# chanchanchan97/ICAFusion

Measured on NVIDIA H100. Metric: 640x512 RGB+IR pairs/sec end-to-end, higher is better.
Workload: dtype f16

## Files before the change

icafusion_b200/_lib.py:

```python
from __future__ import annotations

import ctypes as C
import os

_HERE = os.path.dirname(os.path.abspath(__file__))
LIB_PATH = os.path.join(_HERE, "libicaf_b200.so")

ACT_NONE, ACT_SILU, ACT_GELU = 0, 1, 2
EPI_BIAS_ROW, EPI_ADD_RES, EPI_SCALED_RES, EPI_LN_FOLD, EPI_EMIT_STATS = 1, 2, 4, 8, 16


class ConvGeom(C.Structure):
    _fields_ = [(n, C.c_int) for n in ("B", "Hi", "Wi", "Cin", "Ho", "Wo", "Cout", "kh", "kw", "stride", "pad",
                                       "k_pad", "w_rows", "act", "epi")]


class ConvIO(C.Structure):
    _fields_ = [("x", C.c_void_p), ("x_ld", C.c_int64), ("w", C.c_void_p), ("bias", C.c_void_p),
                ("res", C.c_void_p), ("res_ld", C.c_int64), ("y", C.c_void_p), ("y_ld", C.c_int64),
                ("alpha", C.c_void_p), ("beta", C.c_void_p),
                ("ln_stats", C.c_void_p), ("ln_colsum", C.c_void_p), ("ln_parts", C.c_int), ("ln_eps", C.c_float),
                ("stats_out", C.c_void_p)]


class ConvPlan(C.Structure):
    _fields_ = [(n, C.c_int) for n in ("kernel", "bn", "a_mode", "tile_w", "tile_h", "tiles_x", "tiles_y", "cblk", "halo",
                                       "stages", "splits", "grid_x", "grid_y", "grid_z", "cluster", "smem_bytes",
                                       "work_items", "ctas")]


class LossHyp(C.Structure):
    _fields_ = [(n, C.c_float) for n in ("box", "obj", "cls", "cls_pw", "obj_pw", "anchor_t", "fl_gamma", "gr", "cp", "cn")] + \
               [("balance", C.c_float * 5)]


class AugTile(C.Structure):
    _fields_ = [("rgb", C.c_void_p), ("ir", C.c_void_p)] + \
               [(n, C.c_int) for n in ("H0", "W0", "h", "w", "x1a", "y1a", "x2a", "y2a", "x1b", "y1b", "xtab", "ytab")]


class AugSample(C.Structure):
    _fields_ = [("tile", AugTile * 4)] + [(n, C.c_int) for n in ("ntiles", "canvas", "warp", "flipud", "fliplr", "reserved")] + \
               [("lut", C.c_uint8 * (2 * 3 * 256))]


KERNEL_TC = 0

_vp, _i, _i64, _f = C.c_void_p, C.c_int, C.c_int64, C.c_float
SIGNATURES = {
    "icaf_version": [],
    "icaf_last_error": [],
    "icaf_sm_count": [],
    "icaf_kernel_launches": [],
    "icaf_conv2d_fwd": [C.POINTER(ConvGeom), C.POINTER(ConvIO), _i, _vp],
    "icaf_conv2d_plan": [C.POINTER(ConvGeom), _i, _i, _i, C.POINTER(ConvPlan)],
    "icaf_conv2d_fwd_simt": [C.POINTER(ConvGeom), C.POINTER(ConvIO), _i, _vp],
    "icaf_pack_image": [_vp, _i, _f, _i, _i, _i, _vp, _vp],
    "icaf_pack_image_s2d": [_vp, _i, _f, _i, _i, _i, _vp, _vp],
    "icaf_letterbox": [_vp, _i, _i, _i, _vp, _i, _i, _i, _i, _i, _i, _vp, _vp, _i, _vp],
    "icaf_sppf_pool": [_vp, _i64, _vp, _vp, _vp, _i64, _i, _i, _i, _i, _vp],
    "icaf_upsample2x": [_vp, _i64, _vp, _i64, _i, _i, _i, _i, _vp],
    "icaf_copy_channels": [_vp, _i64, _vp, _i64, _i64, _i, _vp],
    "icaf_prefetch_l2": [_vp, C.c_size_t, _vp],
    "icaf_dmff_pool_tokens": [_vp, _vp, _i64, _vp, _vp, _vp, _vp, _vp, _vp, _vp, _i, _i, _i, _i, _i, _i, _i, _vp],
    "icaf_row_stats": [_vp, _vp, _vp, _vp, _i64, _i, _vp],
    "icaf_layernorm": [_vp, _vp, _vp, _vp, _vp, _vp, _vp, _vp, _i64, _i, _f, _vp],
    "icaf_cross_attention": [_vp, _vp, _vp, _vp, _vp, _vp, _i, _i, _i, _i, _i, _vp],
    "icaf_cross_attention_simt": [_vp, _vp, _vp, _vp, _vp, _vp, _i, _i, _i, _i, _i, _vp],
    "icaf_dmff_upsample_cat": [_vp, _vp, _i, _vp, _vp, _i64, _vp, _i64, _i, _i, _i, _i, _i, _i, _i, _vp],
    "icaf_nms_workspace_bytes": [_i, _i],
    "icaf_nms": [_vp, _i, _i, _i, _f, _f, _i, C.c_uint64, _i, _vp, _vp, _vp, C.c_size_t, _vp],
    "icaf_loss_workspace_bytes": [_i, _i, _i, C.POINTER(C.c_int), C.POINTER(C.c_int), _i, _i],
    "icaf_compute_loss_fwd": [C.POINTER(C.c_void_p), _i, _i, C.POINTER(C.c_int), C.POINTER(C.c_int), _i, _i, _i, _i, _vp, _i,
                              C.POINTER(C.c_float), C.POINTER(LossHyp), _vp, _vp, C.c_size_t, _vp],
    "icaf_compute_loss_bwd": [C.POINTER(C.c_void_p), _i, _i, C.POINTER(C.c_int), C.POINTER(C.c_int), _i, _i, _i, _i, _vp, _i,
                              C.POINTER(C.c_float), C.POINTER(LossHyp), _vp, C.POINTER(C.c_void_p), _vp, C.c_size_t, _vp],
    "icaf_conv2d_wgrad_workspace_bytes": [C.POINTER(ConvGeom)],
    "icaf_conv2d_wgrad": [C.POINTER(ConvGeom), _vp, _i64, _vp, _i64, _vp, _f, _i, _vp, C.c_size_t, _vp],
# ... 21 lines not shown
    "icaf_augment": [_vp, C.c_size_t, _i, _i, _i, _vp, _vp, _vp],
}

_lib = None


class IcafError(RuntimeError):
    pass


def lib() -> C.CDLL:
    global _lib
    if _lib is None:
        if not os.path.exists(LIB_PATH):
            raise IcafError(f"{LIB_PATH} not found -- build it with `python -m icafusion_b200.build`; "
                            "icafusion_b200 has no non-CUDA fallback")
        L = C.CDLL(LIB_PATH)
        for name, argtypes in SIGNATURES.items():
            fn = getattr(L, name)
            fn.argtypes = argtypes
            fn.restype = {"icaf_last_error": C.c_char_p, "icaf_kernel_launches": C.c_longlong,
                          "icaf_nms_workspace_bytes": C.c_size_t, "icaf_loss_workspace_bytes": C.c_size_t,
                          "icaf_conv2d_wgrad_workspace_bytes": C.c_size_t, "icaf_train_workspace_bytes": C.c_size_t,
                          "icaf_cross_attention_bwd_workspace_bytes": C.c_size_t,
                          "icaf_augment_params_bytes": C.c_size_t}.get(name, C.c_int)
        _lib = L
    return _lib


def check(rc: int, what: str = "") -> None:
    if rc != 0:
        msg = lib().icaf_last_error()
        raise IcafError(f"{what or 'icaf call'} failed (code {rc}): {msg.decode() if msg else '?'}")
```

icafusion_b200/csrc/conv_common.cuh:

```cuda
#pragma once
#include "icaf_internal.cuh"

namespace icaf {

constexpr int BM = 128;
constexpr int BK = 64;
constexpr int kLag = 2;
constexpr int kThreads = 288;

enum AMode { A_GATHER = 0, A_TMA2D = 1, A_TMA4D = 2 };

struct ConvProblem {
  const __half* x; const float* bias; const __half* res; __half* y;
  const float* alpha; const float* beta;
  long long x_ld, res_ld, y_ld;
  const float2* ln_stats;
  const float* ln_s;
  float2* stats_out;
};
struct ConvParams {
  ConvProblem p[2];
  int M, N, K, k_pad;
  int B, Hi, Wi, Cin, Ho, Wo, kh, kw, stride, pad;
  int act, epi;
  int a_mode, tw, th, tiles_x, tiles_y;
  int stages;
  int splits;
  int cblk;
  int ln_parts;
  float ln_eps, ln_inv_k;
  int m_tiles, n_tiles, tiles;
  int tma_epi;
};
struct ConvMaps {
  CUtensorMap w[2];
  CUtensorMap a[2];
  CUtensorMap y[2];
  CUtensorMap res[2];
};

__device__ __forceinline__ ConvProblem pick_problem(const ConvParams& P, unsigned z) {
  ConvProblem r;
  r.x = z ? P.p[1].x : P.p[0].x;          r.bias = z ? P.p[1].bias : P.p[0].bias;
  r.res = z ? P.p[1].res : P.p[0].res;    r.y = z ? P.p[1].y : P.p[0].y;
  r.alpha = z ? P.p[1].alpha : P.p[0].alpha; r.beta = z ? P.p[1].beta : P.p[0].beta;
  r.x_ld = z ? P.p[1].x_ld : P.p[0].x_ld; r.res_ld = z ? P.p[1].res_ld : P.p[0].res_ld;
  r.y_ld = z ? P.p[1].y_ld : P.p[0].y_ld;
  r.ln_stats = z ? P.p[1].ln_stats : P.p[0].ln_stats; r.ln_s = z ? P.p[1].ln_s : P.p[0].ln_s;
  r.stats_out = z ? P.p[1].stats_out : P.p[0].stats_out;
  return r;
}

struct TileOrigin { int m0, tb, oy0, ox0; };
__device__ __forceinline__ void tile_origin(const ConvParams& P, int mtile, int& m0, int& tb, int& oy0, int& ox0) {
  m0 = mtile * BM; tb = 0; oy0 = 0; ox0 = 0;
// ... 273 lines not shown
template <int BN>
__device__ __forceinline__ void tma_load_tile(const ConvParams& P, const CUtensorMap* map, uint32_t s, uint32_t bar, int n0,
                                              const TileOrigin& o) {
  const int halves = (BN == 128 && n0 + 64 < P.N) ? 2 : 1;
  const uint32_t half_bytes = P.a_mode == A_TMA4D ? uint32_t(P.tw * P.th) * 128u : uint32_t(kOutHalfBytes);
  mbar_arrive_expect_tx(bar, uint32_t(halves) * half_bytes);
  for (int hh = 0; hh < halves; ++hh) {
    const uint32_t dst = s + uint32_t(hh * kOutHalfBytes);
    if (P.a_mode == A_TMA4D) tma_load_4d(dst, map, bar, n0 + 64 * hh, o.ox0, o.oy0, o.tb);
    else tma_load_2d(dst, map, bar, n0 + 64 * hh, o.m0);
  }
}

struct ConvPlan {
  int kernel;
  int bn;
  unsigned grid_x, grid_y, grid_z, cluster;
  int smem;
  int tiles, m_tiles, n_tiles;
  int sms;
  bool persist;
  bool xm;
  int ctas;
};

}
```

icafusion_b200/csrc/conv_gemm.cu:

```cuda
#include <cstdlib>
#include <cstring>

#include "conv_common.cuh"

namespace icaf {

constexpr int kMaxStages = 10;
template <int BN>
struct SmemLayout {
  static constexpr int kABytes = BM * BK * 2;
  static constexpr int kBBytes = BN * BK * 2;
  static constexpr int kStageBytes = kABytes + kBBytes;
  static constexpr int kPitch = BN + 4;
  static constexpr int kAccBytes = BM * kPitch * 4;
  static constexpr int kTailBytes = 256 + BN * 4 + 1024;
  __host__ __device__ static int region(int stages) { return stages * kStageBytes > kAccBytes ? stages * kStageBytes : kAccBytes; }
  static int total(int stages) { return region(stages) + kTailBytes; }
};


template <int BN, bool kTmaA>
__device__ __forceinline__ void load_stage(const ConvParams& P, int a_mode, uint32_t sa, uint32_t bar, uint32_t bytes,
                                           const CUtensorMap* mw, const CUtensorMap* ma, int kb, int n0, const TileOrigin& o) {
  mbar_arrive_expect_tx(bar, bytes);
// ... 234 lines not shown
    if (elect_one()) {
      const CUtensorMap* mw = bz ? &maps.w[1] : &maps.w[0];
      const CUtensorMap* ma = bz ? &maps.a[1] : &maps.a[0];
      const uint32_t a_bytes = a_mode == A_TMA2D ? L::kABytes : (a_mode == A_TMA4D ? uint32_t(P.tw * P.th) * 128u : 0u);
      const uint32_t bytes = L::kBBytes + a_bytes;
      int s = 0;
      uint32_t ph = 0;
      for (int kb = 0; kb < nkb; ++kb) {
        mbar_wait_quiet(empty_bar(s), ph ^ 1);
        load_stage<BN, false>(P, a_mode, smem_base + s * L::kStageBytes, full_bar(s), bytes, mw, ma, kb_begin + kb, n0, o);
        if (++s == kStages) { s = 0; ph ^= 1; }
      }
      if (tma_epi && has_res) {
        mbar_wait_quiet(empty_bar(s), ph ^ 1);
        tma_load_tile<BN>(P, bz ? &maps.res[1] : &maps.res[0], smem_base + uint32_t(s) * L::kStageBytes, res_bar, n0, o);
      }
    }
    __syncwarp();
    if (splits > 1) { cluster_arrive(); cluster_wait(); cluster_arrive(); cluster_wait(); }
  }
}

constexpr int kPersistThreads = 384;
struct PersistLayout {
  static constexpr int kStageBytes = SmemLayout<128>::kStageBytes;
  static constexpr int kOutBytes = 2 * kOutHalfBytes;
  static constexpr int kPitch = 32 + 4;
  static constexpr int kChunkBytes = BM * kPitch * 4;
  static_assert(kChunkBytes <= kOutBytes, "the XM staged chunk lives in the output tile");
  __host__ __device__ static int bar_off(int stages) { return stages * kStageBytes + 2 * kOutBytes; }
  static int total(int stages) { return bar_off(stages) + 256 + 2 * 128 * 4 + 1024; }
};

struct PersistTile { int z, n0; TileOrigin o; };
__device__ __forceinline__ PersistTile persist_tile(const ConvParams& P, int t) {
  PersistTile pt;
  const int r = t / P.n_tiles;
  const int mtile = r % P.m_tiles;
  pt.n0 = (t - r * P.n_tiles) * 128;
  pt.z = r / P.m_tiles;
  tile_origin(P, mtile, pt.o.m0, pt.o.tb, pt.o.oy0, pt.o.ox0);
  return pt;
}

template <int CC>
__device__ __forceinline__ void stage_chunk(const float (&acc0)[64], const float (&acc1)[64], float* sacc, int w, int l) {
#pragma unroll
  for (int i = 16 * CC; i < 16 * CC + 16; i += 2) {
    const int r = 16 * w + (l >> 2) + 8 * ((i >> 1) & 1), col = 8 * (i >> 2) - 32 * CC + 2 * (l & 3);
    *reinterpret_cast<float2*>(sacc + r * PersistLayout::kPitch + col) = make_float2(acc0[i], acc0[i + 1]);
    *reinterpret_cast<float2*>(sacc + (r + 64) * PersistLayout::kPitch + col) = make_float2(acc1[i], acc1[i + 1]);
  }
}

template <bool XM>
__global__ void __launch_bounds__(kPersistThreads, 1)
conv_gemm_persist_kernel(const ConvParams P, const __grid_constant__ ConvMaps maps) {
  extern __shared__ uint8_t smem_raw[];
  const uint32_t smem_base = (smem_u32(smem_raw) + 1023u) & ~1023u;
  using L = SmemLayout<128>;
  using PL = PersistLayout;
  const int kStages = P.stages;
  const uint32_t bar_off = uint32_t(PL::bar_off(kStages));
  const uint32_t bar_base = smem_base + bar_off;
  auto full_bar = [&](int s) { return bar_base + 8u * s; };
// ... 18 lines not shown
    mbar_init(res_bar(0), 1);
    mbar_init(res_bar(1), 1);
    fence_mbar_init();
  }
  if (tid == 32) {
    tma_prefetch_desc(&maps.w[0]);
    tma_prefetch_desc(&maps.a[0]);
    if (P.tiles > P.m_tiles * P.n_tiles) { tma_prefetch_desc(&maps.w[1]); tma_prefetch_desc(&maps.a[1]); }
    if (!XM) {
      tma_prefetch_desc(&maps.y[0]);
      if (has_res) tma_prefetch_desc(&maps.res[0]);
    }
  }
  __syncthreads();
  pdl_wait();

  if (wg == 0) {
    setmaxnreg_dec<40>();
    if (tid < 32 && elect_one()) {
      const uint32_t a_bytes = a_mode == A_TMA2D ? L::kABytes : uint32_t(P.tw * P.th) * 128u;
      const uint32_t bytes = L::kBBytes + a_bytes;
      int s = 0;
      uint32_t ph = 0;
      for (int tile = blockIdx.x; tile < P.tiles; tile += gridDim.x) {
        const PersistTile pt = persist_tile(P, tile);
        const CUtensorMap* mw = pt.z ? &maps.w[1] : &maps.w[0];
        const CUtensorMap* ma = pt.z ? &maps.a[1] : &maps.a[0];
        for (int kb = 0; kb < nkb; ++kb) {
          mbar_wait_quiet(empty_bar(s), ph ^ 1);
          load_stage<128, true>(P, a_mode, smem_base + s * L::kStageBytes, full_bar(s), bytes, mw, ma, kb, pt.n0, pt.o);
          if (++s == kStages) { s = 0; ph ^= 1; }
        }
      }
    }
    return;
  }

  setmaxnreg_inc<232>();
  const int c = wg - 1;
  const int t = tid & 127, w = t >> 5, l = t & 31;
  const int bar_id = 2 + c;
  const uint32_t sout = smem_base + uint32_t(kStages * L::kStageBytes + c * PL::kOutBytes);
  float* sacc = reinterpret_cast<float*>(smem_gen + kStages * L::kStageBytes + c * PL::kOutBytes);
  float* sbias = reinterpret_cast<float*>(smem_gen + bar_off + 256 + c * 128 * 4);
  for (int tile = blockIdx.x + c * gridDim.x; tile < P.tiles; tile += 2 * gridDim.x) {
    const int j = (tile - int(blockIdx.x)) / int(gridDim.x);
    const PersistTile pt = persist_tile(P, tile);
    const ConvProblem pr = pick_problem(P, pt.z);
    const int n0 = pt.n0;
    const TileOrigin& o = pt.o;
    const float bias_r = (pr.bias && !(P.epi & ICAF_EPI_BIAS_ROW) && n0 + t < P.N) ? __ldg(pr.bias + n0 + t) : 0.f;
    float alpha = 0.f, beta = 1.f;
    if (P.epi & ICAF_EPI_SCALED_RES) { alpha = __ldg(pr.alpha); beta = __ldg(pr.beta); }
    StagedRow sr;
    float rb[4] = {0.f, 0.f, 0.f, 0.f};
    if (XM) {
      staged_row<128, XM>(sr, P, pr, o, t, n0);
    } else {
      fragment_row_bias(rb, P, pr, o, w, l);
      if (t == 0) {
        bulk_wait_group_read<0>();
        if (has_res) tma_load_tile<128>(P, pt.z ? &maps.res[1] : &maps.res[0], sout, res_bar(c), n0, o);
      }
      sbias[t] = bias_r;
      named_bar_sync(bar_id, 128);
    }

    float acc0[64], acc1[64];
#pragma unroll
    for (int i = 0; i < 64; ++i) { acc0[i] = 0.f; acc1[i] = 0.f; }
    auto hand_back = [&](int s) { if (l == 0) mbar_arrive(empty_bar(s)); };
    const int g0 = j * nkb;
    const int s0 = g0 % kStages;
    const uint32_t ph0 = uint32_t(g0 / kStages) & 1u;
    if (j > 0) mbar_wait_quiet(order_bar(c), uint32_t((j >> 1) - (1 - c)) & 1u);
    const int s_last = mma_loop<128>(acc0, acc1, smem_base, kStages, nkb, s0, ph0, full_bar, hand_back);
    if (l == 0) mbar_arrive(order_bar(c ^ 1));
    wgmma_wait<0>();
    hand_back(s_last);

    if constexpr (!XM) {
      if (has_res) mbar_wait_quiet(res_bar(c), uint32_t(j >> 1) & 1u);
      epi_tile_fragments<64>(epi_mode_act<false>(P, has_res), acc0, acc1, sout, sbias, rb, alpha, beta, w, l);
      fence_proxy_async_smem();
      named_bar_sync(bar_id, 128);
      if (t == 0) {
        tma_store_tile<128>(P, pt.z ? &maps.y[1] : &maps.y[0], sout, n0, o);
        if (tile + 2 * int(gridDim.x) >= P.tiles) bulk_wait_group<0>();
      }
      continue;
    }

    const int mode_act = epi_mode_act<XM>(P, has_res);
    const float* arow = sacc + size_t(t) * PL::kPitch;
#pragma unroll 1
    for (int cc = 0; cc < 4; ++cc) {
      named_bar_sync(bar_id, 128);
      if (cc == 0) sbias[t] = bias_r;
      switch (cc) {
        case 0: stage_chunk<0>(acc0, acc1, sacc, w, l); break;
        case 1: stage_chunk<1>(acc0, acc1, sacc, w, l); break;
        case 2: stage_chunk<2>(acc0, acc1, sacc, w, l); break;
        default: stage_chunk<3>(acc0, acc1, sacc, w, l); break;
      }
      named_bar_sync(bar_id, 128);
      const int cb = 32 * cc;
      if (sr.mvalid && n0 + cb < P.N) {
        uint32_t acc[32];
        load_staged(acc, arow);
        epi_staged_chunk<XM>(mode_act, acc, sr, sbias, alpha, beta, cb, n0 + cb, P.N);
      }
// ... 37 lines not shown
  if (!g || n_io < 1 || n_io > 2) return set_error(ICAF_ERR_BAD_ARG, "conv2d: need 1 or 2 problems");
  if (!(g->Cin == 4 || g->Cin % 8 == 0)) return set_error(ICAF_ERR_UNSUPPORTED, "conv2d: Cin must be 4 or a multiple of 8");
  if (g->Cin == 4 && (g->Wi % 2 || g->stride % 2 || g->pad % 2 || g->kw % 2))
    return set_error(ICAF_ERR_UNSUPPORTED, "conv2d: packed-image (Cin=4) path needs even Wi, stride, pad, kw");
  if (g->k_pad % 64 || g->k_pad < g->kh * g->kw * g->Cin) return set_error(ICAF_ERR_BAD_ARG, "conv2d: bad k_pad");
  if (g->w_rows < g->Cout) return set_error(ICAF_ERR_BAD_ARG, "conv2d: w_rows < Cout");
  long long M = (long long)g->B * g->Ho * g->Wo;
  if (M <= 0 || M > 0x7fffffffLL || (long long)g->B * g->Hi * g->Wi > 0x7fffffffLL)
    return set_error(ICAF_ERR_BAD_ARG, "conv2d: size out of range");
  if ((g->epi & (ICAF_EPI_ADD_RES | ICAF_EPI_SCALED_RES)) == (ICAF_EPI_ADD_RES | ICAF_EPI_SCALED_RES))
    return set_error(ICAF_ERR_BAD_ARG, "conv2d: ADD_RES and SCALED_RES are exclusive");
  if ((g->epi & ICAF_EPI_LN_FOLD) && ((g->epi & ~ICAF_EPI_LN_FOLD) != 0 || !(g->act == ICAF_ACT_NONE || g->act == ICAF_ACT_GELU) ||
                                      g->kh != 1 || g->kw != 1 || g->stride != 1 || g->pad != 0))
    return set_error(ICAF_ERR_UNSUPPORTED, "conv2d: LN_FOLD is a linear-layer (1x1) epilogue without residual, activation none / GELU");
  if ((g->epi & ICAF_EPI_EMIT_STATS) && ((g->epi & ~ICAF_EPI_EMIT_STATS) != ICAF_EPI_SCALED_RES || g->act != ICAF_ACT_NONE))
    return set_error(ICAF_ERR_UNSUPPORTED, "conv2d: EMIT_STATS rides on the SCALED_RES epilogue without activation");
  P.M = int(M); P.N = g->Cout; P.K = g->kh * g->kw * g->Cin; P.k_pad = g->k_pad;
  P.B = g->B; P.Hi = g->Hi; P.Wi = g->Wi; P.Cin = g->Cin; P.Ho = g->Ho; P.Wo = g->Wo;
  P.kh = g->kh; P.kw = g->kw; P.stride = g->stride; P.pad = g->pad; P.act = g->act; P.epi = g->epi;
  P.a_mode = A_GATHER; P.tw = P.th = P.tiles_x = P.tiles_y = 0; P.stages = 2; P.splits = 1; P.cblk = 64;
  P.ln_parts = 0; P.ln_eps = 0.f; P.ln_inv_k = 0.f;
  P.m_tiles = P.n_tiles = P.tiles = 0;
  P.tma_epi = 0;
  memset(P.p, 0, sizeof(P.p));
  return ICAF_OK;
}

static int fill_params(const icaf_conv_geom* g, const icaf_conv_io* io, int n_io, ConvParams& P, const __half* (&w)[2]) {
  if (!io) return set_error(ICAF_ERR_BAD_ARG, "conv2d: null io");
  if (int rc = fill_geom(g, n_io, P)) return rc;
  for (int i = 0; i < 2; ++i) {
    const icaf_conv_io& s = io[i < n_io ? i : 0];
    bool need_res = g->epi & (ICAF_EPI_ADD_RES | ICAF_EPI_SCALED_RES);
    if (!s.x || !s.w || !s.y || (need_res && !s.res) || ((g->epi & ICAF_EPI_SCALED_RES) && (!s.alpha || !s.beta)))
      return set_error(ICAF_ERR_BAD_ARG, "conv2d: null pointer");
    if ((reinterpret_cast<uintptr_t>(s.x) & 15) || (reinterpret_cast<uintptr_t>(s.w) & 15) || (s.x_ld % 8 && g->Cin != 4) ||
        (g->Cin == 4 && s.x_ld != 4))
      return set_error(ICAF_ERR_BAD_ARG, "conv2d: x / w must be 16-byte aligned with x_ld a multiple of 8");
    if ((g->epi & ICAF_EPI_LN_FOLD) && (!s.ln_stats || !s.ln_colsum || s.ln_parts < 1 || s.ln_parts > 64))
      return set_error(ICAF_ERR_BAD_ARG, "conv2d: LN_FOLD needs ln_stats, ln_colsum and 1..64 partials per row");
    if ((g->epi & ICAF_EPI_EMIT_STATS) && !s.stats_out) return set_error(ICAF_ERR_BAD_ARG, "conv2d: EMIT_STATS needs stats_out");
    if (i > 0 && (g->epi & ICAF_EPI_LN_FOLD) && (s.ln_parts != io[0].ln_parts || s.ln_eps != io[0].ln_eps))
      return set_error(ICAF_ERR_BAD_ARG, "conv2d: grouped problems must share ln_parts / ln_eps");
    P.p[i] = ConvProblem{(const __half*)s.x, s.bias, need_res ? (const __half*)s.res : nullptr, (__half*)s.y, s.alpha, s.beta,
                         s.x_ld, s.res_ld, s.y_ld,
                         (g->epi & ICAF_EPI_LN_FOLD) ? (const float2*)s.ln_stats : nullptr,
// ... 48 lines not shown
  if (tiles * 2 <= pl.sms && nkb >= 8) {
    splits = int(pl.sms / tiles);
    if (splits > 8) splits = 8;
    if (splits > nkb / 4) splits = nkb / 4;
    if (splits < 1) splits = 1;
  }
  if (splits > 1) {
    const int per = (nkb + splits - 1) / splits;
    if (stages > per) stages = per < 2 ? 2 : per;
    gx *= splits;
  }
  if (stages > kMaxStages || L::total(stages) > kSmemCap)
    return set_error(ICAF_ERR_BAD_ARG, "conv2d(tc): shared-memory plan exceeds the ring / 227 KB");
  P.stages = stages;
  P.splits = splits;
  pl.kernel = ICAF_KERNEL_TC; pl.bn = BN;
  pl.grid_x = gx; pl.grid_y = gy; pl.grid_z = gz; pl.cluster = unsigned(splits);
  pl.smem = L::total(stages);
  pl.tiles = int(tiles); pl.m_tiles = mt; pl.n_tiles = int(gy);
  pl.persist = false; pl.ctas = int(gx * gy * gz);
  return ICAF_OK;
}

static int plan_persist(ConvParams& P, ConvPlan& pl) {
  constexpr int kSmemCap = 227 * 1024;
  int stages = kMaxStages;
  while (stages > 2 && PersistLayout::total(stages) > kSmemCap) --stages;
  if (PersistLayout::total(stages) > kSmemCap)
    return set_error(ICAF_ERR_BAD_ARG, "conv2d(persist): shared-memory plan exceeds 227 KB");
  P.stages = stages;
  P.m_tiles = pl.m_tiles; P.n_tiles = pl.n_tiles; P.tiles = pl.tiles;
  pl.persist = true;
  pl.ctas = pl.tiles < pl.sms ? pl.tiles : pl.sms;
  pl.smem = PersistLayout::total(stages);
  return ICAF_OK;
}

template <int BN>
static int encode_maps(const ConvParams& P, const __half* const (&w)[2], const icaf_conv_geom* g, int n_io, bool out_maps,
                       ConvMaps& maps) {
  memset(&maps, 0, sizeof(maps));
  for (int i = 0; i < n_io; ++i) {
    int rc = encode_tmap_2d(&maps.w[i], w[i], (uint64_t)P.k_pad, (uint64_t)g->w_rows, (uint64_t)P.k_pad * 2, BK, BN);
    if (rc) return rc;
    const ConvProblem& pr = P.p[i];
    if (P.a_mode == A_TMA2D)
      rc = encode_tmap_2d(&maps.a[i], pr.x, (uint64_t)P.Cin, (uint64_t)P.M, (uint64_t)pr.x_ld * 2, BK, BM);
    else if (P.a_mode == A_TMA4D)
      rc = encode_tmap_nhwc(&maps.a[i], pr.x, P.Cin, P.Wi, P.Hi, P.B, pr.x_ld, BK, P.tw * P.stride, P.th * P.stride, P.stride,
                            P.stride);
    if (rc) return rc;
    if (out_maps) {
      auto out_map = [&](CUtensorMap* m, const __half* base, long long ld) {
        return P.a_mode != A_TMA4D ? encode_tmap_2d(m, base, (uint64_t)P.N, (uint64_t)P.M, (uint64_t)ld * 2, 64, BM)
                                   : encode_tmap_nhwc(m, base, P.N, P.Wo, P.Ho, P.B, ld, 64, P.tw, P.th, 1, 1);
      };
      if ((rc = out_map(&maps.y[i], pr.y, pr.y_ld))) return rc;
      if (pr.res && (rc = out_map(&maps.res[i], pr.res, pr.res_ld))) return rc;
    }
  }
  if (n_io == 1) { maps.w[1] = maps.w[0]; maps.a[1] = maps.a[0]; maps.y[1] = maps.y[0]; maps.res[1] = maps.res[0]; }
  return ICAF_OK;
}

template <int BN>
static int launch_conv(const ConvParams& P, const ConvPlan& pl, const __half* const (&w)[2], const icaf_conv_geom* g, int n_io,
                       cudaStream_t st) {
  void (*kernel)(ConvParams, ConvMaps) = pl.xm ? conv_gemm_tc_kernel<BN, true> : conv_gemm_tc_kernel<BN, false>;
  if (pl.persist) kernel = pl.xm ? conv_gemm_persist_kernel<true> : conv_gemm_persist_kernel<false>;
  static bool configured[2][2][kMaxDevices] = {};
  if (int rc = configure_smem(kernel, 227 * 1024, configured[pl.persist][pl.xm], "conv2d: cudaFuncSetAttribute")) return rc;
  ConvMaps maps;
  if (int rc = encode_maps<BN>(P, w, g, n_io, P.tma_epi != 0, maps)) return rc;
  const dim3 grid = pl.persist ? dim3(unsigned(pl.ctas)) : dim3(pl.grid_x, pl.grid_y, pl.grid_z);
  launch_kc(kernel, grid, dim3(pl.persist ? kPersistThreads : kThreads), (size_t)pl.smem, st, pl.cluster, P, maps);
  return check_launch("conv2d_fwd");
}

static int plan_conv(const icaf_conv_geom* g, int n_io, int sms, bool tma_out, ConvParams& P, ConvPlan& pl) {
  memset(&pl, 0, sizeof(pl));
  pl.sms = sms;
  if (sms < 1) return set_error(ICAF_ERR_BAD_ARG, "conv2d: SM count must be positive");
  pl.xm = (P.epi & (ICAF_EPI_LN_FOLD | ICAF_EPI_EMIT_STATS)) != 0;
  plan_a_mode(g, P);
  const long long mt = P.a_mode == A_TMA4D ? (long long)P.B * P.tiles_x * P.tiles_y : (P.M + BM - 1) / BM;
  auto ctas = [&](int bn) { return mt * ((P.N + bn - 1) / bn) * n_io; };
  int bn = 32;
  if (P.N > 64 && ctas(128) >= sms) bn = 128;
  else if (P.N > 32 && ctas(64) >= sms) bn = 64;
  int rc;
  switch (bn) {
    case 128:
      rc = plan_tc<128>(P, n_io, pl);
      if (!rc && (pl.xm || tma_out) && P.a_mode != A_GATHER && P.splits == 1 && pl.tiles > sms) rc = plan_persist(P, pl);
      break;
    case 64: rc = plan_tc<64>(P, n_io, pl); break;
    default: rc = plan_tc<32>(P, n_io, pl); break;
  }
  if (rc) return rc;
  P.tma_epi = !pl.xm && (pl.persist || (tma_out && P.splits == 1 && pl.bn >= 64)) ? 1 : 0;
  return ICAF_OK;
}

}

using namespace icaf;


extern "C" int icaf_conv2d_plan(const icaf_conv_geom* g, int n_io, int sm_count, int pair_mode, icaf_conv_plan* out) {
  if (!out) return set_error(ICAF_ERR_BAD_ARG, "conv2d_plan: null output");
  ConvParams P;
  int rc = fill_geom(g, n_io, P);
  if (rc) return rc;
  ConvPlan pl;
  (void)pair_mode;
  rc = plan_conv(g, n_io, sm_count, true, P, pl);
  if (rc) return rc;
  out->kernel = pl.kernel; out->bn = pl.bn; out->a_mode = P.a_mode;
  out->tile_w = P.tw; out->tile_h = P.th; out->tiles_x = P.tiles_x; out->tiles_y = P.tiles_y;
  out->cblk = P.cblk; out->halo = 0; out->stages = P.stages; out->splits = P.splits;
  out->grid_x = int(pl.grid_x); out->grid_y = int(pl.grid_y); out->grid_z = int(pl.grid_z); out->cluster = int(pl.cluster);
  out->smem_bytes = pl.smem; out->work_items = pl.tiles; out->ctas = pl.ctas;
  return ICAF_OK;
}

extern "C" int icaf_conv2d_fwd(const icaf_conv_geom* g, const icaf_conv_io* io, int n_io, void* stream) {
  ConvParams P;
  const __half* w[2];
  int rc = fill_params(g, io, n_io, P, w);
  if (rc) return rc;
  bool tma_out = true;
  for (int i = 0; i < n_io; ++i) {
    const ConvProblem& pr = P.p[i];
    tma_out = tma_out && (reinterpret_cast<uintptr_t>(pr.y) & 15) == 0 && pr.y_ld % 8 == 0 &&
              (!pr.res || ((reinterpret_cast<uintptr_t>(pr.res) & 15) == 0 && pr.res_ld % 8 == 0));
  }
  ConvPlan pl;
  rc = plan_conv(g, n_io, sm_count_cached(), tma_out, P, pl);
  if (rc) return rc;
  cudaStream_t st = (cudaStream_t)stream;
  switch (pl.bn) {
    case 128: return launch_conv<128>(P, pl, w, g, n_io, st);
    case 64: return launch_conv<64>(P, pl, w, g, n_io, st);
    case 32: return launch_conv<32>(P, pl, w, g, n_io, st);
    default: return set_error(ICAF_ERR_BAD_ARG, "conv2d: the planner produced an unknown tile width");
  }
}

extern "C" int icaf_conv2d_fwd_simt(const icaf_conv_geom* g, const icaf_conv_io* io, int n_io, void* stream) {
  SimtParams S;
  int rc = fill_params(g, io, n_io, S.P, S.w);
  if (rc) return rc;
  long long total = (long long)S.P.M * S.P.N;
  dim3 grid((unsigned)((total + 255) / 256), 1, n_io);
  launch_k(conv_gemm_simt_kernel, dim3(grid), dim3(256), 0, (cudaStream_t)stream, S);
  return check_launch("conv2d_fwd_simt");
}
```

icafusion_b200/ops.py:

```python
from __future__ import annotations

import ctypes as C
from dataclasses import dataclass
from typing import List, Optional, Sequence

import torch

from . import _lib
from ._lib import (ACT_GELU, ACT_NONE, ACT_SILU, EPI_ADD_RES, EPI_BIAS_ROW, EPI_EMIT_STATS, EPI_LN_FOLD,
                   EPI_SCALED_RES)


_PROFILE = None


def launch_count() -> int:
    return int(_lib.lib().icaf_kernel_launches())


class profile:

    def __enter__(self):
        global _PROFILE
        self.records = []
# ... 234 lines not shown
        if tuple(outs[i].shape) != (B, Ho, Wo, p0.cout):
            raise ValueError(f"conv2d: output shape {tuple(outs[i].shape)} != {(B, Ho, Wo, p0.cout)}")
        ios[i].x, ios[i].x_ld = _addr(xs[i]), _check_view(xs[i], "conv2d input")
        ios[i].w = _addr(pk.w)
        ios[i].bias = _addr(pk.bias)
        ios[i].y, ios[i].y_ld = _addr(outs[i]), _check_view(outs[i], "conv2d output")
        if res is not None:
            if tuple(res[i].shape) != (B, Ho, Wo, p0.cout):
                raise ValueError("conv2d: residual shape mismatch")
            ios[i].res, ios[i].res_ld = _addr(res[i]), _check_view(res[i], "conv2d residual")
        if scaled is not None:
            ios[i].alpha, ios[i].beta = _addr(scaled[i][0]), _addr(scaled[i][1])
        if ln_stats is not None:
            st = ln_stats[i]
            if pk.colsum is None or st.dtype != torch.float32 or st.dim() != 3 or st.shape[0] != B * Ho * Wo or st.shape[2] != 2 or \
                    not st.is_contiguous():
                raise ValueError("conv2d: ln_stats must be contiguous fp32 (M, parts, 2) and the filter packed by pack_linear_ln")
            ios[i].ln_stats, ios[i].ln_colsum, ios[i].ln_parts, ios[i].ln_eps = _addr(st), _addr(pk.colsum), st.shape[1], pk.ln_eps
        if stats_out is not None:
            so = stats_out[i]
            if tuple(so.shape) != (B * Ho * Wo, (p0.cout + 31) // 32, 2) or so.dtype != torch.float32 or not so.is_contiguous():
                raise ValueError(f"conv2d: stats_out must be contiguous fp32 {(B * Ho * Wo, (p0.cout + 31) // 32, 2)}")
            ios[i].stats_out = _addr(so)
    fn = _lib.lib().icaf_conv2d_fwd_simt if simt else _lib.lib().icaf_conv2d_fwd
    M = B * Ho * Wo
    kk = p0.kh * p0.kw * p0.cin
    work = {"tag": f"M{M} N{p0.cout} K{kk} k{p0.kh}s{p0.stride} x{n}" + (" +res" if res is not None else ""),
            "flops": 2.0 * M * p0.cout * kk * n,
            "bytes": 2.0 * n * (B * Hi * Wi * p0.cin + M * p0.cout * (2 if res is not None else 1) + p0.cout * kk)}
    work["geom"], work["n_io"] = g, n
    _call("icaf_conv2d_fwd_simt" if simt else "icaf_conv2d_fwd", fn, (C.byref(g), ios, n), work)
    return list(outs)


def linear(xs: Sequence[torch.Tensor], packs: Sequence[PackedConv], outs=None, res=None, scaled=None,
           bias_row: bool = False, simt: bool = False, ln_stats=None, stats_out=None) -> List[torch.Tensor]:
    def as4(t):
        return None if t is None else t.unflatten(0, (1, 1, t.shape[0])) if t.dim() == 2 else t
    o = conv2d([as4(x) for x in xs], packs, None if outs is None else [as4(t) for t in outs],
               None if res is None else [as4(t) for t in res], scaled, bias_row, simt, ln_stats, stats_out)
    return [t[0, 0] for t in o]


def pack_stem_weight(weight: torch.Tensor, bias: Optional[torch.Tensor], act: int, device=None) -> "PackedConv":
    cout, cin, kh, kw = weight.shape
    assert (cin, kh, kw) == (3, 6, 6)
    w = weight.detach().float()
    w4 = torch.cat([w, w.new_zeros(cout, 1, 6, 6)], 1)
    w4 = w4.view(cout, 4, 3, 2, 3, 2)
    ws = w4.permute(0, 3, 5, 1, 2, 4).reshape(cout, 16, 3, 3)
    return pack_conv_weight(ws, bias, 1, 1, act, device)


def pack_image(img: torch.Tensor, scale: float = 1.0, s2d: bool = False) -> torch.Tensor:
    if img.dim() != 4 or img.shape[1] != 3 or not on_device(img):
# ... 415 lines not shown
```

icafusion_b200/trainer.py:

```python
from __future__ import annotations

from typing import Dict, List, Optional

import torch
import torch.nn as nn

from . import _lib
from .common import CrossTransformerBlock
from .loss import ComputeLoss

HYP_SCRATCH = dict(lr0=0.01, momentum=0.937, weight_decay=0.0005, box=0.05, cls=0.5, cls_pw=1.0, obj=1.0, obj_pw=1.0, anchor_t=4.0,
                   fl_gamma=0.0)


def dead_parameters(model: nn.Module) -> List[str]:
    names = []
    for mod_name, m in model.named_modules():
        if isinstance(m, CrossTransformerBlock):
            for sub in ("ln_input", "ln_output", "mlp", "LN1"):
                for k, _ in getattr(m, sub).named_parameters():
                    names.append(f"{mod_name}.{sub}.{k}" if mod_name else f"{sub}.{k}")
    return names


# ... 113 lines not shown
        warmup = (11 if ts.world_size > 1 else 3) if warmup is None else warmup
        saved = {k: v.detach().clone() for k, v in ts.raw_model.state_dict().items()}
        saved_scaler = ts.scaler.state_dict()
        cur = torch.cuda.current_stream(dev)
        side = torch.cuda.Stream(dev)
        side.wait_stream(cur)
        with torch.cuda.stream(side):
            for _ in range(warmup):
                self.seed_ctr += 1
                ts(self.rgb, self.ir, self.tg)
        cur.wait_stream(side)
        torch.cuda.synchronize(dev)
        with torch.no_grad():
            for k, v in ts.raw_model.state_dict().items():
                v.copy_(saved[k])
            for st in ts.optimizer.state.values():
                if st.get("momentum_buffer") is not None:
                    st["momentum_buffer"].zero_()
        if saved_scaler:
            ts.scaler.load_state_dict(saved_scaler)
        self.seed_ctr.zero_()
        ts.zero_grad()
        self.graph = torch.cuda.CUDAGraph()
        with torch.cuda.graph(self.graph):
            self.seed_ctr += 1
            pred = ts.model(self.rgb, self.ir)
            loss, self.items = ts.compute_loss(pred, self.tg)
            if ts.world_size > 1:
                loss = loss * ts.world_size
            self.loss = loss
            ts.scaler.scale(loss).backward()

    def __call__(self, rgb: torch.Tensor, ir: torch.Tensor, targets: torch.Tensor):
        nt = int(targets.shape[0])
        if nt > self.max_targets:
            raise ValueError(f"GraphedTrainStep: {nt} label rows, captured for at most {self.max_targets}")
        self.rgb.copy_(rgb, non_blocking=True)
        self.ir.copy_(ir, non_blocking=True)
        self.tg[:nt].copy_(targets, non_blocking=True)
        if nt < self.max_targets:
            self.tg[nt:, 0] = -1.0
        self.graph.replay()
        self.ts.scaler.step(self.ts.optimizer)
        self.ts.scaler.update()
        if self.ts.ema is not None:
            self.ts.ema.update(self.ts.raw_model)
        return self.loss.detach(), self.items
# ... 4 lines not shown
```

include/icaf_b200.h:

```cpp
#ifndef ICAF_B200_H
#define ICAF_B200_H

#include <stddef.h>
#include <stdint.h>

#ifdef __cplusplus
extern "C" {
#endif

#define ICAF_OK 0
#define ICAF_ERR_BAD_ARG 1
#define ICAF_ERR_UNSUPPORTED 2
#define ICAF_ERR_CUDA 3

#define ICAF_ACT_NONE 0
#define ICAF_ACT_SILU 1
#define ICAF_ACT_GELU 2

#define ICAF_EPI_BIAS_ROW 1
#define ICAF_EPI_ADD_RES 2
#define ICAF_EPI_SCALED_RES 4
#define ICAF_EPI_LN_FOLD 8
#define ICAF_EPI_EMIT_STATS 16

// ... 22 lines not shown
  const float* beta;
  const float* ln_stats;
  const float* ln_colsum;
  int ln_parts;
  float ln_eps;
  float* stats_out;
} icaf_conv_io;

int icaf_conv2d_fwd(const icaf_conv_geom* g, const icaf_conv_io* io, int n_io, void* stream);

#define ICAF_KERNEL_TC 0
typedef struct {
  int kernel;
  int bn;
  int a_mode;
  int tile_w, tile_h, tiles_x, tiles_y;
  int cblk;
  int halo;
  int stages, splits;
  int grid_x, grid_y, grid_z, cluster;
  int smem_bytes;
  int work_items;
  int ctas;
} icaf_conv_plan;
int icaf_conv2d_plan(const icaf_conv_geom* g, int n_io, int sm_count, int pair_mode, icaf_conv_plan* out);

int icaf_conv2d_fwd_simt(const icaf_conv_geom* g, const icaf_conv_io* io, int n_io, void* stream);

int icaf_pack_image(const void* src, int src_dtype, float scale, int B, int H, int W, void* dst, void* stream);

int icaf_letterbox(const void* src, int B, int H0, int W0, void* dst, int H, int W, int top, int left, int new_h, int new_w,
                   const int* xtab, const int* ytab, int pad_value, void* stream);

int icaf_pack_image_s2d(const void* src, int src_dtype, float scale, int B, int H, int W, void* dst, void* stream);

int icaf_sppf_pool(const void* x, int64_t x_ld, void* y1, void* y2, void* y3, int64_t y_ld, int B, int H, int W,
                   int C, void* stream);

int icaf_upsample2x(const void* x, int64_t x_ld, void* y, int64_t y_ld, int B, int H, int W, int C, void* stream);

int icaf_prefetch_l2(const void* ptr, size_t bytes, void* stream);

int icaf_copy_channels(const void* x, int64_t x_ld, void* y, int64_t y_ld, int64_t pixels, int C, void* stream);

int icaf_dmff_pool_tokens(const void* x_vis, const void* x_ir, int64_t x_ld, const void* pos_vis, const void* pos_ir,
                          const float* mix, void* tok_vis, void* tok_ir, float* stats_vis, float* stats_ir, int B, int H,
                          int W, int C, int nh, int nw, int n_pad, void* stream);

// ... 111 lines not shown
```

Before: 1532.

## Split-K the persistent conv's tail wave across idle CTAs with fp32 workspace reduction

In the persistent TMA conv kernel, the remainder tiles that would leave most SMs idle in the last wave are split along K across several CTAs. Each CTA writes partial fp32 accumulators to a global workspace and takes a ticket with an atomic, and the last arriver sums the partials before running the epilogue. The intent is to remove last-wave load imbalance. The cost is extra global traffic, fences and a new workspace that is cached per stream and zeroed after graph capture. The training graph capture is also moved onto the side stream.

Measured after the change: 1534, median of 6. No clear change (+0.1%).

```diff
diff --git a/icafusion_b200/_lib.py b/icafusion_b200/_lib.py
--- a/icafusion_b200/_lib.py
+++ b/icafusion_b200/_lib.py
@@ -26,7 +26,7 @@
 class ConvPlan(C.Structure):
     _fields_ = [(n, C.c_int) for n in ("kernel", "bn", "a_mode", "tile_w", "tile_h", "tiles_x", "tiles_y", "cblk", "halo",
                                        "stages", "splits", "grid_x", "grid_y", "grid_z", "cluster", "smem_bytes",
-                                       "work_items", "ctas")]
+                                       "work_items", "ctas", "tail_tiles", "tail_splits")]
 
 
 class LossHyp(C.Structure):
@@ -54,6 +54,9 @@
     "icaf_kernel_launches": [],
     "icaf_conv2d_fwd": [C.POINTER(ConvGeom), C.POINTER(ConvIO), _i, _vp],
     "icaf_conv2d_plan": [C.POINTER(ConvGeom), _i, _i, _i, C.POINTER(ConvPlan)],
+    "icaf_conv2d_plan_ws": [C.POINTER(ConvGeom), _i, _i, C.POINTER(ConvPlan)],
+    "icaf_conv2d_workspace_bytes": [C.POINTER(ConvGeom), _i],
+    "icaf_conv2d_fwd_ws": [C.POINTER(ConvGeom), C.POINTER(ConvIO), _i, _vp, C.c_size_t, _vp],
     "icaf_conv2d_fwd_simt": [C.POINTER(ConvGeom), C.POINTER(ConvIO), _i, _vp],
     "icaf_pack_image": [_vp, _i, _f, _i, _i, _i, _vp, _vp],
     "icaf_pack_image_s2d": [_vp, _i, _f, _i, _i, _i, _vp, _vp],
@@ -121,6 +124,7 @@
             fn.restype = {"icaf_last_error": C.c_char_p, "icaf_kernel_launches": C.c_longlong,
                           "icaf_nms_workspace_bytes": C.c_size_t, "icaf_loss_workspace_bytes": C.c_size_t,
                           "icaf_conv2d_wgrad_workspace_bytes": C.c_size_t, "icaf_train_workspace_bytes": C.c_size_t,
+                          "icaf_conv2d_workspace_bytes": C.c_size_t,
                           "icaf_cross_attention_bwd_workspace_bytes": C.c_size_t,
                           "icaf_augment_params_bytes": C.c_size_t}.get(name, C.c_int)
         _lib = L
diff --git a/icafusion_b200/csrc/conv_common.cuh b/icafusion_b200/csrc/conv_common.cuh
--- a/icafusion_b200/csrc/conv_common.cuh
+++ b/icafusion_b200/csrc/conv_common.cuh
@@ -31,6 +31,10 @@
   float ln_eps, ln_inv_k;
   int m_tiles, n_tiles, tiles;
   int tma_epi;
+  int whole_tiles;
+  int tail_units, tail_splits;
+  uint32_t* tail_tickets;
+  float* tail_slots;
 };
 struct ConvMaps {
   CUtensorMap w[2];
@@ -350,6 +354,7 @@
   bool persist;
   bool xm;
   int ctas;
-};
-
-}
+  size_t ws_bytes;
+};
+
+}
diff --git a/icafusion_b200/csrc/conv_gemm.cu b/icafusion_b200/csrc/conv_gemm.cu
--- a/icafusion_b200/csrc/conv_gemm.cu
+++ b/icafusion_b200/csrc/conv_gemm.cu
@@ -280,6 +280,10 @@
 }
 
 constexpr int kPersistThreads = 384;
+constexpr int kTailSlotFloats = BM * 128;
+constexpr int kMaxTailSplits = 4;
+constexpr int kMinTailBlocks = 18;
+inline size_t tail_ticket_bytes(int sms) { return (size_t(sms) * 4 + 15) / 16 * 16; }
 struct PersistLayout {
   static constexpr int kStageBytes = SmemLayout<128>::kStageBytes;
   static constexpr int kOutBytes = 2 * kOutHalfBytes;
@@ -299,6 +303,16 @@
   pt.z = r / P.m_tiles;
   tile_origin(P, mtile, pt.o.m0, pt.o.tb, pt.o.oy0, pt.o.ox0);
   return pt;
+}
+
+struct PersistUnit { int tile, kb0, nkb; };
+__device__ __forceinline__ PersistUnit persist_unit(const ConvParams& P, int b, int G, int j, int nkb) {
+  const int tile = b + j * G;
+  if (tile < P.whole_tiles) return PersistUnit{tile, 0, nkb};
+  if (tile - G >= P.whole_tiles || b >= P.tail_units) return PersistUnit{-1, 0, 0};
+  const int k = P.tail_splits, part = b % k;
+  const int kb0 = nkb * part / k;
+  return PersistUnit{P.whole_tiles + b / k, kb0, nkb * (part + 1) / k - kb0};
 }
 
 template <int CC>
@@ -363,13 +377,15 @@
       const uint32_t bytes = L::kBBytes + a_bytes;
       int s = 0;
       uint32_t ph = 0;
-      for (int tile = blockIdx.x; tile < P.tiles; tile += gridDim.x) {
-        const PersistTile pt = persist_tile(P, tile);
+      for (int j = 0;; ++j) {
+        const PersistUnit u = persist_unit(P, blockIdx.x, gridDim.x, j, nkb);
+        if (u.tile < 0) break;
+        const PersistTile pt = persist_tile(P, u.tile);
         const CUtensorMap* mw = pt.z ? &maps.w[1] : &maps.w[0];
         const CUtensorMap* ma = pt.z ? &maps.a[1] : &maps.a[0];
-        for (int kb = 0; kb < nkb; ++kb) {
+        for (int kb = 0; kb < u.nkb; ++kb) {
           mbar_wait_quiet(empty_bar(s), ph ^ 1);
-          load_stage<128, true>(P, a_mode, smem_base + s * L::kStageBytes, full_bar(s), bytes, mw, ma, kb, pt.n0, pt.o);
+          load_stage<128, true>(P, a_mode, smem_base + s * L::kStageBytes, full_bar(s), bytes, mw, ma, u.kb0 + kb, pt.n0, pt.o);
           if (++s == kStages) { s = 0; ph ^= 1; }
         }
       }
@@ -384,9 +400,10 @@
   const uint32_t sout = smem_base + uint32_t(kStages * L::kStageBytes + c * PL::kOutBytes);
   float* sacc = reinterpret_cast<float*>(smem_gen + kStages * L::kStageBytes + c * PL::kOutBytes);
   float* sbias = reinterpret_cast<float*>(smem_gen + bar_off + 256 + c * 128 * 4);
-  for (int tile = blockIdx.x + c * gridDim.x; tile < P.tiles; tile += 2 * gridDim.x) {
-    const int j = (tile - int(blockIdx.x)) / int(gridDim.x);
-    const PersistTile pt = persist_tile(P, tile);
+  for (int j = c;; j += 2) {
+    const PersistUnit u = persist_unit(P, blockIdx.x, gridDim.x, j, nkb);
+    if (u.tile < 0) break;
+    const PersistTile pt = persist_tile(P, u.tile);
     const ConvProblem pr = pick_problem(P, pt.z);
     const int n0 = pt.n0;
     const TileOrigin& o = pt.o;
@@ -415,10 +432,48 @@
     const int s0 = g0 % kStages;
     const uint32_t ph0 = uint32_t(g0 / kStages) & 1u;
     if (j > 0) mbar_wait_quiet(order_bar(c), uint32_t((j >> 1) - (1 - c)) & 1u);
-    const int s_last = mma_loop<128>(acc0, acc1, smem_base, kStages, nkb, s0, ph0, full_bar, hand_back);
+    const int s_last = mma_loop<128>(acc0, acc1, smem_base, kStages, u.nkb, s0, ph0, full_bar, hand_back);
     if (l == 0) mbar_arrive(order_bar(c ^ 1));
     wgmma_wait<0>();
     hand_back(s_last);
+
+    if (!XM && int(blockIdx.x) + j * int(gridDim.x) >= P.whole_tiles) {
+      const int k = P.tail_splits, ti = int(blockIdx.x) / k;
+      constexpr int kSlot4 = kTailSlotFloats / 4;
+      float4* slot = reinterpret_cast<float4*>(P.tail_slots) + size_t(blockIdx.x) * kSlot4;
+#pragma unroll
+      for (int q = 0; q < 16; ++q) {
+        slot[q * 128 + t] = make_float4(acc0[4 * q], acc0[4 * q + 1], acc0[4 * q + 2], acc0[4 * q + 3]);
+        slot[(16 + q) * 128 + t] = make_float4(acc1[4 * q], acc1[4 * q + 1], acc1[4 * q + 2], acc1[4 * q + 3]);
+      }
+      __threadfence();
+      named_bar_sync(bar_id, 128);
+      volatile uint32_t* sticket = reinterpret_cast<uint32_t*>(smem_gen + bar_off + 8 * (2 * kMaxStages + 4)) + c;
+      if (t == 0) {
+        uint32_t* ctr = P.tail_tickets + ti;
+        const uint32_t tk = atomicAdd(ctr, 1u);
+        if (tk == uint32_t(k - 1)) *ctr = 0u;
+        __threadfence();
+        *sticket = tk;
+      }
+      named_bar_sync(bar_id, 128);
+      if (*sticket != uint32_t(k - 1)) {
+        if (has_res) mbar_wait_quiet(res_bar(c), uint32_t(j >> 1) & 1u);
+        if (t == 0) bulk_wait_group<0>();
+        continue;
+      }
+#pragma unroll
+      for (int i = 0; i < 64; ++i) { acc0[i] = 0.f; acc1[i] = 0.f; }
+#pragma unroll 1
+      for (int off = ti * k * kSlot4 + t; off < (ti + 1) * k * kSlot4; off += kSlot4) {
+#pragma unroll
+        for (int q = 0; q < 32; ++q) {
+          const float4 x = __ldcg(reinterpret_cast<const float4*>(P.tail_slots) + off + q * 128);
+          float* a = q < 16 ? acc0 + 4 * q : acc1 + 4 * (q - 16);
+          a[0] += x.x; a[1] += x.y; a[2] += x.z; a[3] += x.w;
+        }
+      }
+    }
 
     if constexpr (!XM) {
       if (has_res) mbar_wait_quiet(res_bar(c), uint32_t(j >> 1) & 1u);
@@ -427,7 +482,7 @@
       named_bar_sync(bar_id, 128);
       if (t == 0) {
         tma_store_tile<128>(P, pt.z ? &maps.y[1] : &maps.y[0], sout, n0, o);
-        if (tile + 2 * int(gridDim.x) >= P.tiles) bulk_wait_group<0>();
+        if (persist_unit(P, blockIdx.x, gridDim.x, j + 2, nkb).tile < 0) bulk_wait_group<0>();
       }
       continue;
     }
@@ -511,6 +566,7 @@
   P.ln_parts = 0; P.ln_eps = 0.f; P.ln_inv_k = 0.f;
   P.m_tiles = P.n_tiles = P.tiles = 0;
   P.tma_epi = 0;
+  P.whole_tiles = 0; P.tail_units = 0; P.tail_splits = 1; P.tail_tickets = nullptr; P.tail_slots = nullptr;
   memset(P.p, 0, sizeof(P.p));
   return ICAF_OK;
 }
@@ -605,7 +661,7 @@
   return ICAF_OK;
 }
 
-static int plan_persist(ConvParams& P, ConvPlan& pl) {
+static int plan_persist(ConvParams& P, ConvPlan& pl, bool tail_split) {
   constexpr int kSmemCap = 227 * 1024;
   int stages = kMaxStages;
   while (stages > 2 && PersistLayout::total(stages) > kSmemCap) --stages;
@@ -613,9 +669,18 @@
     return set_error(ICAF_ERR_BAD_ARG, "conv2d(persist): shared-memory plan exceeds 227 KB");
   P.stages = stages;
   P.m_tiles = pl.m_tiles; P.n_tiles = pl.n_tiles; P.tiles = pl.tiles;
+  P.whole_tiles = pl.tiles;
   pl.persist = true;
   pl.ctas = pl.tiles < pl.sms ? pl.tiles : pl.sms;
   pl.smem = PersistLayout::total(stages);
+  const int r = pl.tiles % pl.ctas;
+  int k = r > 0 ? pl.ctas / r : 0;
+  if (k > kMaxTailSplits) k = kMaxTailSplits;
+  if (k > P.k_pad / BK / kMinTailBlocks) k = P.k_pad / BK / kMinTailBlocks;
+  if (tail_split && !pl.xm && k >= 2) {
+    P.whole_tiles = pl.tiles - r; P.tail_units = r * k; P.tail_splits = k;
+    pl.ws_bytes = tail_ticket_bytes(pl.sms) + size_t(r) * k * kTailSlotFloats * sizeof(float);
+  }
   return ICAF_OK;
 }
 
@@ -660,7 +725,7 @@
   return check_launch("conv2d_fwd");
 }
 
-static int plan_conv(const icaf_conv_geom* g, int n_io, int sms, bool tma_out, ConvParams& P, ConvPlan& pl) {
+static int plan_conv(const icaf_conv_geom* g, int n_io, int sms, bool tma_out, bool tail_split, ConvParams& P, ConvPlan& pl) {
   memset(&pl, 0, sizeof(pl));
   pl.sms = sms;
   if (sms < 1) return set_error(ICAF_ERR_BAD_ARG, "conv2d: SM count must be positive");
@@ -675,7 +740,7 @@
   switch (bn) {
     case 128:
       rc = plan_tc<128>(P, n_io, pl);
-      if (!rc && (pl.xm || tma_out) && P.a_mode != A_GATHER && P.splits == 1 && pl.tiles > sms) rc = plan_persist(P, pl);
+      if (!rc && (pl.xm || tma_out) && P.a_mode != A_GATHER && P.splits == 1 && pl.tiles > sms) rc = plan_persist(P, pl, tail_split);
       break;
     case 64: rc = plan_tc<64>(P, n_io, pl); break;
     default: rc = plan_tc<32>(P, n_io, pl); break;
@@ -690,24 +755,43 @@
 using namespace icaf;
 
 
-extern "C" int icaf_conv2d_plan(const icaf_conv_geom* g, int n_io, int sm_count, int pair_mode, icaf_conv_plan* out) {
+static int conv2d_plan(const icaf_conv_geom* g, int n_io, int sm_count, bool tail_split, icaf_conv_plan* out) {
   if (!out) return set_error(ICAF_ERR_BAD_ARG, "conv2d_plan: null output");
   ConvParams P;
   int rc = fill_geom(g, n_io, P);
   if (rc) return rc;
   ConvPlan pl;
-  (void)pair_mode;
-  rc = plan_conv(g, n_io, sm_count, true, P, pl);
+  rc = plan_conv(g, n_io, sm_count, true, tail_split, P, pl);
   if (rc) return rc;
   out->kernel = pl.kernel; out->bn = pl.bn; out->a_mode = P.a_mode;
   out->tile_w = P.tw; out->tile_h = P.th; out->tiles_x = P.tiles_x; out->tiles_y = P.tiles_y;
   out->cblk = P.cblk; out->halo = 0; out->stages = P.stages; out->splits = P.splits;
   out->grid_x = int(pl.grid_x); out->grid_y = int(pl.grid_y); out->grid_z = int(pl.grid_z); out->cluster = int(pl.cluster);
   out->smem_bytes = pl.smem; out->work_items = pl.tiles; out->ctas = pl.ctas;
+  out->tail_tiles = P.tail_units / P.tail_splits; out->tail_splits = P.tail_splits;
   return ICAF_OK;
 }
 
-extern "C" int icaf_conv2d_fwd(const icaf_conv_geom* g, const icaf_conv_io* io, int n_io, void* stream) {
+extern "C" int icaf_conv2d_plan(const icaf_conv_geom* g, int n_io, int sm_count, int pair_mode, icaf_conv_plan* out) {
+  (void)pair_mode;
+  return conv2d_plan(g, n_io, sm_count, false, out);
+}
+
+extern "C" int icaf_conv2d_plan_ws(const icaf_conv_geom* g, int n_io, int sm_count, icaf_conv_plan* out) {
+  return conv2d_plan(g, n_io, sm_count, true, out);
+}
+
+extern "C" size_t icaf_conv2d_workspace_bytes(const icaf_conv_geom* g, int n_io) {
+  const int sms = sm_count_cached();
+  if (!g) return tail_ticket_bytes(sms) + size_t(sms) * kTailSlotFloats * sizeof(float);
+  ConvParams P;
+  ConvPlan pl;
+  if (fill_geom(g, n_io, P) || plan_conv(g, n_io, sms, true, true, P, pl)) return 0;
+  return pl.ws_bytes;
+}
+
+static int conv2d_fwd(const icaf_conv_geom* g, const icaf_conv_io* io, int n_io, void* workspace, size_t workspace_bytes,
+                      void* stream) {
   ConvParams P;
   const __half* w[2];
   int rc = fill_params(g, io, n_io, P, w);
@@ -719,8 +803,14 @@
               (!pr.res || ((reinterpret_cast<uintptr_t>(pr.res) & 15) == 0 && pr.res_ld % 8 == 0));
   }
   ConvPlan pl;
-  rc = plan_conv(g, n_io, sm_count_cached(), tma_out, P, pl);
+  rc = plan_conv(g, n_io, sm_count_cached(), tma_out, workspace != nullptr, P, pl);
   if (rc) return rc;
+  if (pl.ws_bytes) {
+    if (workspace_bytes < pl.ws_bytes || (reinterpret_cast<uintptr_t>(workspace) & 15))
+      return set_error(ICAF_ERR_BAD_ARG, "conv2d: workspace smaller than icaf_conv2d_workspace_bytes or not 16-byte aligned");
+    P.tail_tickets = static_cast<uint32_t*>(workspace);
+    P.tail_slots = reinterpret_cast<float*>(static_cast<char*>(workspace) + tail_ticket_bytes(pl.sms));
+  }
   cudaStream_t st = (cudaStream_t)stream;
   switch (pl.bn) {
     case 128: return launch_conv<128>(P, pl, w, g, n_io, st);
@@ -728,6 +818,15 @@
     case 32: return launch_conv<32>(P, pl, w, g, n_io, st);
     default: return set_error(ICAF_ERR_BAD_ARG, "conv2d: the planner produced an unknown tile width");
   }
+}
+
+extern "C" int icaf_conv2d_fwd(const icaf_conv_geom* g, const icaf_conv_io* io, int n_io, void* stream) {
+  return conv2d_fwd(g, io, n_io, nullptr, 0, stream);
+}
+
+extern "C" int icaf_conv2d_fwd_ws(const icaf_conv_geom* g, const icaf_conv_io* io, int n_io, void* workspace, size_t workspace_bytes,
+                                  void* stream) {
+  return conv2d_fwd(g, io, n_io, workspace, workspace_bytes, stream);
 }
 
 extern "C" int icaf_conv2d_fwd_simt(const icaf_conv_geom* g, const icaf_conv_io* io, int n_io, void* stream) {
diff --git a/icafusion_b200/ops.py b/icafusion_b200/ops.py
--- a/icafusion_b200/ops.py
+++ b/icafusion_b200/ops.py
@@ -280,15 +280,36 @@
             if tuple(so.shape) != (B * Ho * Wo, (p0.cout + 31) // 32, 2) or so.dtype != torch.float32 or not so.is_contiguous():
                 raise ValueError(f"conv2d: stats_out must be contiguous fp32 {(B * Ho * Wo, (p0.cout + 31) // 32, 2)}")
             ios[i].stats_out = _addr(so)
-    fn = _lib.lib().icaf_conv2d_fwd_simt if simt else _lib.lib().icaf_conv2d_fwd
     M = B * Ho * Wo
     kk = p0.kh * p0.kw * p0.cin
     work = {"tag": f"M{M} N{p0.cout} K{kk} k{p0.kh}s{p0.stride} x{n}" + (" +res" if res is not None else ""),
             "flops": 2.0 * M * p0.cout * kk * n,
             "bytes": 2.0 * n * (B * Hi * Wi * p0.cin + M * p0.cout * (2 if res is not None else 1) + p0.cout * kk)}
     work["geom"], work["n_io"] = g, n
-    _call("icaf_conv2d_fwd_simt" if simt else "icaf_conv2d_fwd", fn, (C.byref(g), ios, n), work)
+    if simt:
+        _call("icaf_conv2d_fwd_simt", _lib.lib().icaf_conv2d_fwd_simt, (C.byref(g), ios, n), work)
+    else:
+        ws = None if _DRY is not None else _conv_workspace(xs[0].device)
+        _call("icaf_conv2d_fwd", _lib.lib().icaf_conv2d_fwd_ws,
+              (C.byref(g), ios, n, _ptr(ws), C.c_size_t(0 if ws is None else ws.numel() * ws.element_size())), work)
     return list(outs)
+
+
+_CONV_WS = {}
+
+
+def _conv_workspace(dev: torch.device) -> torch.Tensor:
+    st = torch.cuda.current_stream(dev)
+    key = (dev, st.cuda_stream)
+    capturing = torch.cuda.is_current_stream_capturing()
+    ent = _CONV_WS.get(key)
+    if ent is None:
+        nbytes = int(_lib.lib().icaf_conv2d_workspace_bytes(None, 0))
+        ent = _CONV_WS[key] = [torch.zeros((nbytes + 15) // 16, 4, dtype=torch.float32, device=dev), capturing]
+    elif ent[1] and not capturing:
+        ent[0].zero_()
+        ent[1] = False
+    return ent[0]
 
 
 def linear(xs: Sequence[torch.Tensor], packs: Sequence[PackedConv], outs=None, res=None, scaled=None,
diff --git a/icafusion_b200/trainer.py b/icafusion_b200/trainer.py
--- a/icafusion_b200/trainer.py
+++ b/icafusion_b200/trainer.py
@@ -159,7 +159,7 @@
         self.seed_ctr.zero_()
         ts.zero_grad()
         self.graph = torch.cuda.CUDAGraph()
-        with torch.cuda.graph(self.graph):
+        with torch.cuda.graph(self.graph, stream=side):
             self.seed_ctr += 1
             pred = ts.model(self.rgb, self.ir)
             loss, self.items = ts.compute_loss(pred, self.tg)
diff --git a/include/icaf_b200.h b/include/icaf_b200.h
--- a/include/icaf_b200.h
+++ b/include/icaf_b200.h
@@ -68,8 +68,14 @@
   int smem_bytes;
   int work_items;
   int ctas;
+  int tail_tiles, tail_splits;
 } icaf_conv_plan;
 int icaf_conv2d_plan(const icaf_conv_geom* g, int n_io, int sm_count, int pair_mode, icaf_conv_plan* out);
+int icaf_conv2d_plan_ws(const icaf_conv_geom* g, int n_io, int sm_count, icaf_conv_plan* out);
+
+size_t icaf_conv2d_workspace_bytes(const icaf_conv_geom* g, int n_io);
+int icaf_conv2d_fwd_ws(const icaf_conv_geom* g, const icaf_conv_io* io, int n_io, void* workspace, size_t workspace_bytes,
+                       void* stream);
 
 int icaf_conv2d_fwd_simt(const icaf_conv_geom* g, const icaf_conv_io* io, int n_io, void* stream);
 
```
